# pangenome/sweepga

Hardware: AMD Instinct MI355X
Metric: PAF mappings/sec through plane-sweep+scaffold filter, 1/2/4/8 MI355X (higher is better)
Workload: dtype u32 coordinates, f64 scores; 1 GPU; BASELINE.json configs[3] (synthetic 100 M mappings across 10 k (q,t) groups, 100-genome pangenome shape; S-pan in SURVEY.md 8d): 100000000 mappings per GPU over 9900 genome-pair groups (100 single-chromosome genomes), pipeline=default; flags=(defaults), mappings_per_gpu=100000000, groups_per_gpu=9900

## Files before the change

### sweepga_amd/csrc/swg_pair.hip

```cpp
#include <cmath>
#include <type_traits>

#include "swg_scaffold_internal.h"

namespace swg_scaf {
namespace {

constexpr uint32_t PAIR_CELL = WALK_CHUNK;
constexpr uint32_t PAIR_S_MAX = 1024, PAIR_M_MAX = 4096, PAIR_L_MAX = 32768, PAIR_XL_MAX = uint32_t(1) << 18;
constexpr uint32_t PAIR_XL_CELLS = PAIR_XL_MAX / PAIR_CELL;
constexpr uint32_t PAIR_HASH_MAX = 65536;
constexpr uint32_t PF_NOT_GROUPED = 1, PF_RUN_OVERFLOW = 2, PF_TOO_LONG = 4, PF_FALLBACK = 8;

struct PairRun {
  uint32_t a, n;
};
struct PairInfo {
  uint32_t m;
  uint32_t m_plus;
  uint32_t M;
  uint32_t first_alive;
  uint32_t first_mem[2];
  uint32_t q, t;
};
struct PairSum {
  uint32_t n_pass;
  uint32_t n_kept;
  uint32_t minmem;
  uint32_t base;
};
struct PairCounters {
  uint32_t n_runs;
  uint32_t flags;
  uint32_t n_class[4];
  uint32_t n_chunks;
  uint32_t n_long;
  unsigned long long n_alive, n_members, n_heads, n_kept, n_out;
};

__device__ __forceinline__ void lds_barrier() {
  __builtin_amdgcn_fence(__ATOMIC_RELEASE, "wavefront");
  __builtin_amdgcn_s_waitcnt(0xc07f);
  __builtin_amdgcn_s_barrier();
  __builtin_amdgcn_fence(__ATOMIC_ACQUIRE, "wavefront");
}

template <int NT>
__device__ __forceinline__ uint32_t block_excl_sum(uint32_t v, uint32_t* ws, uint32_t* total) {
  const int lane = threadIdx.x & 63, w = threadIdx.x >> 6;
  uint32_t inc = v;
#pragma unroll
  for (int d = 1; d < 64; d <<= 1) {
    const uint32_t t = __shfl_up(inc, d, 64);
    if (lane >= d) inc += t;
  }
  if (NT == 64) {
    *total = __shfl(inc, 63, 64);
    return inc - v;
  }
  lds_barrier();
  if (lane == 63) ws[w] = inc;
  lds_barrier();
  uint32_t off = 0, tot = 0;
#pragma unroll
  for (int k = 0; k < NT / 64; ++k) {
    const uint32_t x = ws[k];
    off += k < w ? x : 0u;
// ... 132 lines not shown
    uint32_t h = (uint32_t)((key * 0x9e3779b97f4a7c15ull) >> 32) & tmask;
    for (;;) {
      const unsigned long long old = atomicCAS(&table[h], ~0ull, key);
      if (old == ~0ull) break;
      if (old == key) {
        atomicOr(&C->flags, PF_NOT_GROUPED);
        break;
      }
      h = (h + 1) & tmask;
    }
  }
  unsigned long long mk[4];
#pragma unroll
  for (int c = 0; c < 4; ++c) {
    mk[c] = __ballot(cls == c);
    if (lane == 0) s_cnt[wv][c] = (uint32_t)__popcll(mk[c]);
  }
  __syncthreads();
  if (threadIdx.x < 4) {
    const int c = threadIdx.x;
    const uint32_t tot = s_cnt[0][c] + s_cnt[1][c] + s_cnt[2][c] + s_cnt[3][c];
    s_base[c] = tot ? atomicAdd(&C->n_class[c], tot) : 0u;
  }
  __syncthreads();
  if (cls >= 0) {
    uint32_t o = s_base[cls];
    for (int w2 = 0; w2 < wv; ++w2) o += s_cnt[w2][cls];
    const unsigned long long m = cls == 0 ? mk[0] : (cls == 1 ? mk[1] : (cls == 2 ? mk[2] : mk[3]));
    class_list[(size_t)cls * cap + o + (uint32_t)__popcll(m & ((1ull << lane) - 1ull))] = k;
  }
}

constexpr int ORDER_NT = 1024, ORDER_BINS = 256;
__global__ __launch_bounds__(ORDER_NT) void pair_order_kernel(const PairRun* __restrict__ runs, uint32_t* __restrict__ class_list, uint32_t cap,
                                                              uint32_t* __restrict__ tmp, uint32_t cap_tmp,
                                                              const PairCounters* __restrict__ C) {
  __shared__ uint32_t bin_at[ORDER_BINS];
  const int tid = threadIdx.x, cls = 2 + (int)blockIdx.x;
  if (C->flags) return;
  const uint32_t cnt = C->n_class[cls];
  if (cnt < 2u || cnt > cap_tmp || cnt > cap) return;
  const uint32_t lo = cls == 2 ? PAIR_M_MAX : PAIR_L_MAX, width = (cls == 2 ? PAIR_L_MAX : PAIR_XL_MAX) - lo;
  uint32_t* const list = class_list + (size_t)cls * cap;
  uint32_t* const t = tmp + (size_t)blockIdx.x * cap_tmp;
  auto bin_of = [&](uint32_t len) -> uint32_t {
    const uint32_t b = (uint32_t)(((uint64_t)(len - lo - 1u) * ORDER_BINS) / width);
    return (uint32_t)ORDER_BINS - 1u - (b < (uint32_t)ORDER_BINS ? b : (uint32_t)ORDER_BINS - 1u);
  };
  for (int b = tid; b < ORDER_BINS; b += ORDER_NT) bin_at[b] = 0u;
  __syncthreads();
  for (uint32_t i = tid; i < cnt; i += ORDER_NT) {
    const uint32_t k = list[i];
    t[i] = k;
    atomicAdd(&bin_at[bin_of(runs[k].n)], 1u);
  }
  __syncthreads();
  if (tid < 64) {
    constexpr int PER = ORDER_BINS / 64;
    uint32_t v[PER], s = 0;
#pragma unroll
    for (int j = 0; j < PER; ++j) {
      v[j] = bin_at[tid * PER + j];
      s += v[j];
    }
    uint32_t inc = s;
#pragma unroll
    for (int d = 1; d < 64; d <<= 1) {
      const uint32_t x = __shfl_up(inc, d, 64);
      if (tid >= d) inc += x;
    }
    uint32_t o = inc - s;
#pragma unroll
    for (int j = 0; j < PER; ++j) {
      bin_at[tid * PER + j] = o;
      o += v[j];
    }
  }
  __syncthreads();
  for (uint32_t i = tid; i < cnt; i += ORDER_NT) {
    const uint32_t k = t[i];
    list[atomicAdd(&bin_at[bin_of(runs[k].n)], 1u)] = k;
  }
}

__global__ __launch_bounds__(256) void pair_hash_kernel(uint32_t n, const uint32_t* __restrict__ q_id, const uint32_t* __restrict__ t_id,
                                                        unsigned long long* __restrict__ table, uint32_t tmask,
                                                        uint32_t* __restrict__ count, uint32_t* __restrict__ slot_of) {
  const uint32_t i = blockIdx.x * 256u + threadIdx.x;
  if (i >= n) return;
  const unsigned long long key = (((unsigned long long)q_id[i] << 32) | t_id[i]) + 1ull;
  uint32_t h = (uint32_t)((key * 0x9e3779b97f4a7c15ull) >> 32) & tmask;
  for (;;) {
    unsigned long long old = __hip_atomic_load(&table[h], __ATOMIC_RELAXED, __HIP_MEMORY_SCOPE_AGENT);
    if (old == 0ull) {
      old = atomicCAS(&table[h], 0ull, key);
      if (old == 0ull) old = key;
    }
    if (old == key) break;
    h = (h + 1) & tmask;
  }
  slot_of[i] = h;
  atomicAdd(&count[h], 1u);
}
__global__ __launch_bounds__(256) void pair_slots_kernel(uint32_t tsize, const uint32_t* __restrict__ count, uint32_t* __restrict__ start,
                                                         PairRun* __restrict__ runs, uint32_t* __restrict__ class_list, uint32_t cap,
                                                         PairCounters* __restrict__ C, uint32_t* __restrict__ cursor) {
  const uint32_t h = blockIdx.x * 256u + threadIdx.x;
  const uint32_t c = h < tsize ? count[h] : 0u;
  if (!c) return;
// ... 56 lines not shown
  uint32_t b = (uint32_t)f;
  const uint32_t top = nb - 1u;
  b = b < top ? b : top;
  return off + b;
}

struct PairSortArgs {
  const uint32_t *q_id, *t_id, *q_start, *q_end, *t_start, *t_end, *matches, *block_len;
  const double* identity;
  const uint8_t* strand;
  const uint8_t *alive_in, *member_in;
  uint64_t min_block;
  int keep_self;
  double min_identity;
  int check_degenerate;
  uint64_t max_gap;
  const PairRun* runs;
  const uint32_t* list;
  const uint32_t* perm;
  const uint32_t* orig;
  uint8_t* code;
  uint32_t *s_qs, *s_qe, *s_ts, *s_te, *s_m, *s_b, *s_idx, *pred;
  PairInfo* info;
  SpecBlock* chunks;
  uint32_t cap_chunks;
  int chunks_by_place;
  uint32_t* long_list;
  uint32_t cap_long;
  PairCounters* C;
  PairTable gl_first;
  const uint32_t* seq_genome_last;
};

__device__ void emit_chunks(const PairSortArgs& A, uint32_t rk_run, uint32_t a, uint32_t m, uint32_t m_plus, const uint32_t* cellmin, int n_cell) {
  uint32_t prev = NONE, count = 0, n_long = 0, prev2 = NONE;
  const bool mp_pending = m_plus > 0 && m_plus < m;
  auto for_starts = [&](auto&& f) {
    bool pend = mp_pending;
    for (int c = 0; c < n_cell; ++c) {
      const uint32_t v = cellmin[c];
      if (v == NONE) continue;
      if (pend && m_plus <= v) {
        if (m_plus < v) f(m_plus);
        pend = false;
      }
      f(v);
    }
    if (pend) f(m_plus);
  };
  for_starts([&](uint32_t v) {
    ++count;
    if (prev2 != NONE && v - prev2 >= LABEL_CAP_ELEMS) ++n_long;
    prev2 = v;
  });
  if (prev2 != NONE && m - prev2 >= LABEL_CAP_ELEMS) ++n_long;
  const uint32_t slot = A.chunks_by_place ? a / PAIR_CELL + 2u * rk_run : atomicAdd(&A.C->n_chunks, count);
  uint32_t lslot = n_long ? atomicAdd(&A.C->n_long, n_long) : 0u;
  if (slot + count > A.cap_chunks || (n_long && lslot + n_long > A.cap_long)) {
    atomicOr(&A.C->flags, PF_FALLBACK);
    return;
  }
  uint32_t k = 0;
  auto emit = [&](uint32_t b, uint32_t e) {
    SpecBlock d;
    d.bb = a + b;
    d.be = a + e;
    d.ue = d.be;
    d.pad = b >= m_plus ? 1u : 0u;
    if (e - b >= LABEL_CAP_ELEMS) A.long_list[lslot++] = slot + k;
    A.chunks[slot + k++] = d;
  };
  for_starts([&](uint32_t v) {
    if (prev != NONE) emit(prev, v);
    prev = v;
  });
  if (prev != NONE) emit(prev, m);
}
template <int NT, int E>
__device__ __forceinline__ void unit_starts(const uint32_t (&qs)[E], const uint32_t (&qe)[E], uint32_t mb, uint32_t base, uint32_t m_plus,
                                            uint64_t max_gap, uint64_t* ws64, uint32_t* cellmin, uint64_t* carry_max) {
  const uint32_t p0 = (uint32_t)threadIdx.x * E;
  uint64_t tmax = 0;
#pragma unroll
  for (int e = 0; e < E; ++e)
    if (p0 + e < mb) {
      const uint64_t c = ((uint64_t)(base + p0 + e >= m_plus ? 1u : 0u) << 32) | qe[e];
      tmax = c > tmax ? c : tmax;
    }
  uint64_t tot;
  uint64_t prev = block_excl_max<NT>(tmax, ws64, &tot);
  prev = prev > *carry_max ? prev : *carry_max;
#pragma unroll
  for (int e = 0; e < E; ++e)
    if (p0 + e < mb) {
      const uint32_t pa = base + p0 + e;
      uint64_t lim = (prev & 0xffffffffull) + max_gap;
      if (lim < max_gap) lim = ~0ull;
      if (pa == 0 || pa == m_plus || (uint64_t)qs[e] > lim) atomicMin(&cellmin[pa / PAIR_CELL], pa);
      const uint64_t c = ((uint64_t)(pa >= m_plus ? 1u : 0u) << 32) | qe[e];
      prev = c > prev ? c : prev;
    }
  *carry_max = tot > *carry_max ? tot : *carry_max;
}
template <int E>
__device__ __forceinline__ void read_block(const uint32_t* lds, uint32_t (&out)[E]) {
  static_assert(E % 4 == 0, "whole 16-byte reads");
  const uint4* v = reinterpret_cast<const uint4*>(lds) + (size_t)threadIdx.x * (E / 4);
#pragma unroll
  for (int j = 0; j < E / 4; ++j) {
// ... 26 lines not shown
  constexpr int CAP = NT * ES, NREC = NT * ER, MAXB = 16, H = 8;
  constexpr int NCELL = (NREC + (int)PAIR_CELL - 1) / (int)PAIR_CELL;
  static_assert(ER <= 32 && ER % H == 0 && ES % 4 == 0 && NREC <= 65536, "record masks are 32 bits wide, indices 16");
  static_assert(NBIN >= 2 && NBIN <= 4096, "each strand needs a coarse bin of its own (the members are ordered strand first)");
  constexpr size_t O_K = 0, O_I = O_K + (size_t)CAP * 4, O_RR = O_I + (size_t)CAP * sizeof(IT), O_CNT = lds_align_up(O_RR + (size_t)CAP * 2, 4),
                   O_BINS = O_CNT + (size_t)NBK * 4, O_BLO = O_BINS + (size_t)NBIN * 4, O_CELL = O_BLO + (size_t)(MAXB + 1) * 4,
                   O_WS64 = lds_align_up(O_CELL + (size_t)NCELL * 4, 8), O_WS = O_WS64 + (size_t)(NT / 64 + 1) * 8,
                   O_SH = O_WS + (size_t)(NT / 64 + 1) * 4;
  static_assert(O_SH + 13 * 4 <= pair_sort_lds_bytes<NT, ES, ER, NBK, NBIN, PERM>(), "LDS block of the work-group");
  static_assert(O_CNT - O_I >= (size_t)CAP * 4 && O_I % 16 == 0, "B1 holds CAP words, read 16 bytes at a time");
  uint32_t* const K = reinterpret_cast<uint32_t*>(lds_raw + O_K);
  IT* const I = reinterpret_cast<IT*>(lds_raw + O_I);
  uint16_t* const RR = reinterpret_cast<uint16_t*>(lds_raw + O_RR);
  uint32_t* const B0 = K;
  uint32_t* const B1 = reinterpret_cast<uint32_t*>(lds_raw + O_I);
  uint32_t* const cnt = reinterpret_cast<uint32_t*>(lds_raw + O_CNT);
  uint32_t* const bins = reinterpret_cast<uint32_t*>(lds_raw + O_BINS);
  uint32_t* const b_lo = reinterpret_cast<uint32_t*>(lds_raw + O_BLO);
  uint32_t* const cellmin = reinterpret_cast<uint32_t*>(lds_raw + O_CELL);
  uint64_t* const ws64 = reinterpret_cast<uint64_t*>(lds_raw + O_WS64);
  uint32_t* const ws = reinterpret_cast<uint32_t*>(lds_raw + O_WS);
  uint32_t* const sh_cnt = reinterpret_cast<uint32_t*>(lds_raw + O_SH);
  uint32_t* const sh_kmin = sh_cnt + 4;
  uint32_t* const sh_kmax = sh_cnt + 6;
  uint32_t* const sh_first = sh_cnt + 8;
  uint32_t& sh_nb = sh_cnt[11];
  uint32_t& sh_bad = sh_cnt[12];
#ifdef SWG_PAIR_TIMING
  unsigned long long pt_last = wall_clock64();
#endif
  const int tid = threadIdx.x;
  const PairRun run = A.runs[rk_run];
  const uint32_t a = run.a, n = run.n;
  if (tid < 4) sh_cnt[tid] = 0;
  if (tid < 2) {
    sh_kmin[tid] = 0xffffffffu;
    sh_kmax[tid] = 0;
  }
  if (tid < 3) sh_first[tid] = NONE;
  if (tid == 0) sh_bad = 0;
  for (int c = tid; c < NCELL; c += NT) cellmin[c] = NONE;
  for (int b = tid; b < NBIN; b += NT) bins[b] = 0;
  lds_barrier();
  auto fresh_tid = [&]() -> uint32_t {
    uint32_t t = (uint32_t)tid;
    asm volatile("" : "+v"(t));
    return t;
  };
  uint32_t tid_v = (uint32_t)tid, n_v = n;
  auto rec_index = [&](int e) -> uint32_t {
    const uint32_t li = tid_v + (uint32_t)e * NT;
    const uint32_t lc = li < n_v ? li : 0u;
    return PERM ? A.perm[a + lc] : lc;
  };
  const uint32_t cb = PERM ? 0u : a;
  const uint32_t* c_qs = A.q_start + cb;
  const uint32_t* c_qe = A.q_end + cb;
  const uint32_t* c_ts = A.t_start + cb;
  const uint32_t* c_te = A.t_end + cb;
  const uint32_t* c_m = A.matches + cb;
  const uint32_t* c_b = A.block_len + cb;
  const uint8_t* c_st = A.strand + cb;
  const double* c_id = A.identity ? A.identity + cb : nullptr;
  const uint8_t* c_alive = A.alive_in ? A.alive_in + cb : nullptr;
  const uint8_t* c_member = A.member_in ? A.member_in + cb : nullptr;
  uint32_t* o_qs = A.s_qs + a;
// ... 437 lines not shown
      unit_starts<NT, ES>(qs_r, qe_r, mb, base, m_plus, A.max_gap, ws64, cellmin, &carry_max);
    }
    column(c_ts, B0, after_prev, B1, o_qe);
    lds_barrier();
    PT_STAMP(7);
    column(c_te, B1, after_prev, B0, o_ts);
    uint32_t ts_r[ES];
    read_block<ES>(B0, ts_r);
    lds_barrier();
    PT_STAMP(8);
    if (A.s_m) {
      column(c_m, B0, after_prev, B1, o_te);
    } else {
      store_column(B1, o_te);
    }
    {
      uint32_t te_r[ES];
      read_block<ES>(B1, te_r);
#pragma unroll
      for (int e = 0; e < ES; ++e) degenerate |= (uint32_t)tid * ES + e < mb && ts_r[e] >= te_r[e];
    }
    PT_STAMP(9);
    if (A.s_m) {
      lds_barrier();
      column(c_b, B1, after_prev, B0, o_m);
      lds_barrier();
      PT_STAMP(10);
      store_column(B1, o_b);
    }
    base += mb;
    PT_STAMP(11);
  }
  if (A.check_degenerate && __any(degenerate) && (tid & 63) == 0) atomicOr(&A.C->flags, PF_FALLBACK);
  if (tid == 0) emit_chunks(A, rk_run, a, m, m_plus, cellmin, NCELL);
  PT_STAMP(12);
}

template <int NT, int E, int NBK>
constexpr size_t pair_sort_xl_lds_bytes() {
  return (size_t)NT * E * 12 + (size_t)NBK * 4 + 4096 * 4 + 129 * 4 + (size_t)PAIR_XL_CELLS * 4 + (size_t)(NT / 64 + 1) * 12 + 16 * 4 + 128;
}
template <int NT, int E, int NBK>
__device__ __forceinline__ void pair_sort_xl_body(const PairSortArgs& A, const uint32_t rk_run, char* lds_raw) {
  constexpr int CAP = NT * E;
  constexpr int NBIN = 4096, MAXB = 128, U = 8;
  constexpr size_t O_K = 0, O_QE = O_K + (size_t)CAP * 4, O_I = O_QE + (size_t)CAP * 4, O_CNT = O_I + (size_t)CAP * 4,
                   O_BINS = O_CNT + (size_t)NBK * 4, O_BLO = O_BINS + (size_t)NBIN * 4, O_CELL = O_BLO + (size_t)(MAXB + 1) * 4,
                   O_WS64 = lds_align_up(O_CELL + (size_t)PAIR_XL_CELLS * 4, 8), O_WS = O_WS64 + (size_t)(NT / 64 + 1) * 8,
                   O_SH = O_WS + (size_t)(NT / 64 + 1) * 4;
  static_assert(O_SH + 13 * 4 <= pair_sort_xl_lds_bytes<NT, E, NBK>(), "LDS block of the work-group");
  uint32_t* const K = reinterpret_cast<uint32_t*>(lds_raw + O_K);
  uint32_t* const QE = reinterpret_cast<uint32_t*>(lds_raw + O_QE);
  uint32_t* const I = reinterpret_cast<uint32_t*>(lds_raw + O_I);
  uint32_t* const cnt = reinterpret_cast<uint32_t*>(lds_raw + O_CNT);
  uint32_t* const bins = reinterpret_cast<uint32_t*>(lds_raw + O_BINS);
  uint32_t* const b_lo = reinterpret_cast<uint32_t*>(lds_raw + O_BLO);
  uint32_t* const cellmin = reinterpret_cast<uint32_t*>(lds_raw + O_CELL);
  uint64_t* const ws64 = reinterpret_cast<uint64_t*>(lds_raw + O_WS64);
  uint32_t* const ws = reinterpret_cast<uint32_t*>(lds_raw + O_WS);
  uint32_t* const sh_cnt = reinterpret_cast<uint32_t*>(lds_raw + O_SH);
  uint32_t* const sh_kmin = sh_cnt + 4;
  uint32_t* const sh_kmax = sh_cnt + 6;
  uint32_t* const sh_first = sh_cnt + 8;
  uint32_t& sh_nb = sh_cnt[11];
  uint32_t& sh_bad = sh_cnt[12];
#ifdef SWG_PAIR_TIMING
  unsigned long long pt_last = wall_clock64();
// ... 319 lines not shown
      }
#pragma unroll
      for (int e = 0; e < E; ++e) {
        const uint32_t p = (uint32_t)tid + (uint32_t)e * NT;
        if (p >= mb) continue;
        const uint32_t o = a + base + p, qs = K[p];
        QE[p] = qe[e];
        A.s_qs[o] = qs;
        A.s_idx[o] = a + li[e];
        A.pred[o] = NONE;
        A.s_qe[o] = qe[e];
        A.s_ts[o] = ts[e];
        A.s_te[o] = te[e];
        if (A.s_m) {
          A.s_m[o] = mm[e];
          A.s_b[o] = bb[e];
        }
        degenerate |= qs >= qe[e] || ts[e] >= te[e];
      }
    }
    __syncthreads();
    PT_STAMP(7);
    {
      uint32_t qs_r[E], qe_r[E];
      read_block<E>(K, qs_r);
      read_block<E>(QE, qe_r);
      unit_starts<NT, E>(qs_r, qe_r, mb, base, m_plus, A.max_gap, ws64, cellmin, &carry_max);
    }
    base += mb;
    __syncthreads();
    PT_STAMP(8);
  }
  if (A.check_degenerate && __any(degenerate) && (tid & 63) == 0) atomicOr(&A.C->flags, PF_FALLBACK);
  if (tid == 0) emit_chunks(A, rk_run, a, m, m_plus, cellmin, (int)PAIR_XL_CELLS);
  PT_STAMP(9);
}

template <int NT, int ES, int ER, int NBK, int NBIN, bool PERM>
__global__ __launch_bounds__(NT) void pair_sort_kernel(PairSortArgs A) {
  __shared__ __attribute__((aligned(16))) char raw[pair_sort_lds_bytes<NT, ES, ER, NBK, NBIN, PERM>()];
  pair_sort_body<NT, ES, ER, NBK, NBIN, PERM>(A, A.list[blockIdx.x], raw);
}
constexpr size_t PAIR_BIG_LDS = pair_sort_lds_bytes<1024, 16, 32, 4096, 1024, false>() > pair_sort_xl_lds_bytes<1024, 8, 4096>()
                                    ? pair_sort_lds_bytes<1024, 16, 32, 4096, 1024, false>()
                                    : pair_sort_xl_lds_bytes<1024, 8, 4096>();
static_assert(PAIR_BIG_LDS <= 160 * 1024, "LDS of a CU");
__global__ __launch_bounds__(1024) void pair_sort_big_kernel(PairSortArgs A, const uint32_t* __restrict__ list_xl, uint32_t n_xl) {
  __shared__ __attribute__((aligned(16))) char raw[PAIR_BIG_LDS];
  if (blockIdx.x < n_xl)
    pair_sort_xl_body<1024, 8, 4096>(A, list_xl[blockIdx.x], raw);
  else
    pair_sort_body<1024, 16, 32, 4096, 1024, false>(A, A.list[blockIdx.x - n_xl], raw);
}

__global__ __launch_bounds__(1024) void pair_totals_kernel(uint32_t n_runs, const PairInfo* __restrict__ info, const PairSum* __restrict__ sum,
                                                           const uint32_t* __restrict__ n_out_pair, PairCounters* __restrict__ C) {
  __shared__ unsigned long long part[16][4];
  unsigned long long v[4] = {0, 0, 0, 0};
  const bool finished = !(C->flags & PF_FALLBACK);
  for (uint32_t k = blockIdx.x * 1024u + threadIdx.x; k < n_runs; k += gridDim.x * 1024u) {
    const PairInfo pi = info[k];
    v[0] += pi.M;
    v[1] += pi.m;
    if (finished) {
      v[2] += pi.M ? sum[k].n_kept : 0u;
      v[3] += n_out_pair[k];
    }
  }
#pragma unroll
  for (int j = 0; j < 4; ++j) {
#pragma unroll
    for (int o = 32; o > 0; o >>= 1) v[j] += __shfl_xor(v[j], o, 64);
    if ((threadIdx.x & 63) == 0) part[threadIdx.x >> 6][j] = v[j];
  }
  __syncthreads();
// ... 986 lines not shown
  const uint32_t n = (uint32_t)n64;
  hipStream_t st = ctx->stream;
  uint64_t* key = swg_alloc<uint64_t>(ctx, n);
  uint64_t* key2 = swg_alloc<uint64_t>(ctx, n);
  uint32_t* val = swg_alloc<uint32_t>(ctx, n);
  uint32_t* val2 = swg_alloc<uint32_t>(ctx, n);
  uint32_t* c4[8];
  for (auto& p : c4) p = swg_alloc<uint32_t>(ctx, n);
  double* c_id = r->identity ? swg_alloc<double>(ctx, n) : nullptr;
  uint8_t* c_st = swg_alloc<uint8_t>(ctx, n);
  SWG_CHECK_ARENA(ctx);
  SWG_LAUNCH(ctx, "pair_group_key", pair_group_key_kernel<<<(n + 255) / 256, 256, 0, st>>>(n, r->q_id, r->t_id, r->n_seq, key, val));
  SWG_KERNEL_CHECK(ctx);
  SWG_TRY(swg_radix_sort_pairs(ctx, &key, &val, &key2, &val2, n, 0, key_bits));
  SWG_LAUNCH(ctx, "pair_group_gather", pair_group_gather_kernel<<<(n + 255) / 256, 256, 0, st>>>(n, val, r->q_id, r->t_id, r->q_start, r->q_end, r->t_start, r->t_end,
                                                                                       r->matches, r->block_len, r->identity, r->strand, c4[0], c4[1], c4[2],
                                                                                       c4[3], c4[4], c4[5], c4[6], c4[7], c_id, c_st));
  SWG_KERNEL_CHECK(ctx);
  *copy = *r;
  copy->q_id = c4[0]; copy->t_id = c4[1]; copy->q_start = c4[2]; copy->q_end = c4[3]; copy->t_start = c4[4]; copy->t_end = c4[5];
  copy->matches = c4[6]; copy->block_len = c4[7]; copy->identity = c_id; copy->strand = c_st;
  *perm_out = val;
  *ok = 1;
  return SWG_OK;
}
int pair_ungroup_results(swg_ctx* ctx, uint64_t n, const uint32_t* perm, const uint8_t* st, const uint32_t* ch, uint8_t* status_out, uint32_t* chain_out) {
  SWG_LAUNCH(ctx, "pair_ungroup", pair_ungroup_kernel<<<(unsigned)((n + 255) / 256), 256, 0, ctx->stream>>>((uint32_t)n, perm, st, ch, status_out, chain_out));
  SWG_KERNEL_CHECK(ctx);
  return SWG_OK;
}

namespace {

}

int pair_plan(swg_ctx* ctx, const swg_records* r, const swg_config* cfg, PairPlan* plan) {
  *plan = PairPlan{};
  if (!pair_path_wanted()) return SWG_OK;
  const uint64_t n64 = r->n;
  if (n64 < 2 || n64 >= (uint64_t(1) << 31)) return SWG_OK;
  const uint32_t n = (uint32_t)n64;
  hipStream_t st = ctx->stream;
  static const bool dbg = getenv("SWG_DEBUG") != nullptr;
  const swg_arena_mark mark0 = swg_arena_save(ctx);
  const bool by_hash = n <= PAIR_HASH_MAX;
  bool plain = cfg != nullptr;
  if (cfg) {
    const bool sf_limited = cfg->scaffold_filter_mode == SWG_MODE_ONE_TO_ONE || cfg->scaffold_filter_mode == SWG_MODE_ONE_TO_MANY ||
                            cfg->scaffold_max_per_query != 0 || cfg->scaffold_max_per_target != 0;
    const bool mf_limited = cfg->mapping_filter_mode == SWG_MODE_ONE_TO_ONE || cfg->mapping_filter_mode == SWG_MODE_ONE_TO_MANY ||
                            cfg->mapping_max_per_query != 0 || cfg->mapping_max_per_target != 0;
    plain = !sf_limited && !mf_limited && (cfg->scaffolds_only || cfg->scaffold_max_deviation == 0);
  }
  static const uint32_t per_pair_env = getenv("SWG_PAIR_MIN_AVG") && atoi(getenv("SWG_PAIR_MIN_AVG")) > 0 ? (uint32_t)atoi(getenv("SWG_PAIR_MIN_AVG")) : 0u;
  const uint32_t per_pair = per_pair_env ? per_pair_env : (plain ? 96u : 192u);
  const uint32_t cap = by_hash ? (n < 8192u ? n : 8192u) : (n / per_pair > 8192u ? n / per_pair : 8192u);
  uint32_t tsize = 1;
  while (tsize < 2 * (by_hash ? n : cap)) tsize <<= 1;
  PairCounters* C = nullptr;
  PairRun* runs = swg_alloc<PairRun>(ctx, cap);
  uint32_t* class_list = swg_alloc<uint32_t>(ctx, (size_t)4 * cap);
  uint32_t* perm = nullptr;
  if (by_hash) {
    char* z = static_cast<char*>(swg_arena_alloc(ctx, (size_t)tsize * 12 + sizeof(PairCounters) + 8));
    uint32_t* slot_of = swg_alloc<uint32_t>(ctx, n);
    uint32_t* start = swg_alloc<uint32_t>(ctx, tsize);
// ... 1 lines not shown
    SWG_CHECK_ARENA(ctx);
    unsigned long long* table = reinterpret_cast<unsigned long long*>(z);
    uint32_t* count = reinterpret_cast<uint32_t*>(z + (size_t)tsize * 8);
    C = reinterpret_cast<PairCounters*>(z + (size_t)tsize * 12);
    uint32_t* cursor = reinterpret_cast<uint32_t*>(z + (size_t)tsize * 12 + sizeof(PairCounters));
    SWG_HIP(ctx, hipMemsetAsync(z, 0, (size_t)tsize * 12 + sizeof(PairCounters) + 8, st));
    SWG_LAUNCH(ctx, "pair_hash", pair_hash_kernel<<<(n + 255) / 256, 256, 0, st>>>(n, r->q_id, r->t_id, table, tsize - 1, count, slot_of));
    SWG_LAUNCH(ctx, "pair_slots", pair_slots_kernel<<<(tsize + 255) / 256, 256, 0, st>>>(tsize, count, start, runs, class_list, cap, C, cursor));
    SWG_LAUNCH(ctx, "pair_perm", pair_perm_kernel<<<(n + 255) / 256, 256, 0, st>>>(n, slot_of, start, perm));
    SWG_KERNEL_CHECK(ctx);
  } else {
    C = swg_alloc<PairCounters>(ctx, 1);
    const uint32_t n_words = (n + 63) / 64;
    unsigned long long* bitmap = swg_alloc<unsigned long long>(ctx, n_words + 1);
    uint32_t* wcnt = swg_alloc<uint32_t>(ctx, n_words + 1);
    uint32_t* wpre = swg_alloc<uint32_t>(ctx, n_words + 1);
    uint32_t* starts = swg_alloc<uint32_t>(ctx, (size_t)cap + 2);
    unsigned long long* table = swg_alloc<unsigned long long>(ctx, tsize);
    uint64_t* d_nr = swg_alloc<uint64_t>(ctx, 1);
    static const bool order_knob = !(getenv("SWG_PAIR_ORDER") && atoi(getenv("SWG_PAIR_ORDER")) == 0);
    const uint32_t cap_tmp = n / PAIR_M_MAX + 1u < cap ? n / PAIR_M_MAX + 1u : cap;
    uint32_t* order_tmp = order_knob ? swg_alloc<uint32_t>(ctx, (size_t)2 * cap_tmp) : nullptr;
    SWG_CHECK_ARENA(ctx);
    SWG_HIP(ctx, hipMemsetAsync(C, 0, sizeof(PairCounters), st));
    SWG_HIP(ctx, hipMemsetAsync(table, 0xff, (size_t)tsize * 8, st));
    SWG_LAUNCH(ctx, "pair_boundary", pair_boundary_kernel<<<(n + 1023) / 1024, 256, 0, st>>>(n, r->q_id, r->t_id, bitmap, wcnt));
    SWG_KERNEL_CHECK(ctx);
    SWG_TRY(swg_exclusive_scan_u32(ctx, wcnt, wpre, n_words, d_nr));
    SWG_LAUNCH(ctx, "pair_runs", pair_starts_kernel<<<(n_words + 255) / 256, 256, 0, st>>>(n, n_words, bitmap, wpre, d_nr, cap, starts));
    SWG_KERNEL_CHECK(ctx);
    SWG_LAUNCH(ctx, "pair_runs", pair_runs_kernel<<<(cap + 255) / 256, 256, 0, st>>>(n, cap, d_nr, starts, r->q_id, r->t_id, table, tsize - 1, runs, class_list, C));
    SWG_KERNEL_CHECK(ctx);
    if (order_knob && n > PAIR_M_MAX) {
      SWG_LAUNCH(ctx, "pair_order", pair_order_kernel<<<2, ORDER_NT, 0, st>>>(runs, class_list, cap, order_tmp, cap_tmp, C));
      SWG_KERNEL_CHECK(ctx);
    }
  }
  uint64_t h[4];
  static_assert(sizeof(PairCounters) >= 32, "the first four words are read back");
  SWG_TRY(swg_read_scalars(ctx, reinterpret_cast<const uint64_t*>(C), h, 3));
  const uint32_t n_runs = (uint32_t)h[0], flags = (uint32_t)(h[0] >> 32);
  if (flags || n_runs == 0) {
    if (dbg) fprintf(stderr, "[swg] pair path: not applicable (%u runs, flags %u)\n", n_runs, flags);
    plan->not_grouped = !by_hash && (flags & (PF_NOT_GROUPED | PF_RUN_OVERFLOW)) && !(flags & PF_TOO_LONG);
    swg_arena_restore(ctx, mark0);
    return SWG_OK;
  }
  if ((uint64_t)n / n_runs > PAIR_L_MAX) {
    if (dbg) fprintf(stderr, "[swg] pair path: %u pairs of %llu records on average: left to the global-sort stage\n", n_runs, (unsigned long long)n / n_runs);
    swg_arena_restore(ctx, mark0);
    return SWG_OK;
  }
  plan->valid = 1;
  plan->by_hash = by_hash;
  plan->n_runs = n_runs;
  plan->ncls[0] = (uint32_t)h[1];
  plan->ncls[1] = (uint32_t)(h[1] >> 32);
  plan->ncls[2] = (uint32_t)h[2];
  plan->ncls[3] = (uint32_t)(h[2] >> 32);
  plan->cap = cap;
  plan->counters = C;
  plan->runs = runs;
  plan->class_list = class_list;
  plan->perm = perm;
  if (dbg)
    fprintf(stderr, "[swg] pair path: %u pairs (%u / %u / %u / %u by size class)%s\n", n_runs, plan->ncls[0], plan->ncls[1], plan->ncls[2],
            plan->ncls[3], by_hash ? ", found through the hash table" : "");
  return SWG_OK;
}

int scaffold_stage_pairs(swg_ctx* ctx, const swg_records* r, const swg_config* cfg, const uint8_t* alive, const uint8_t* member,
                         bool sweep_assumed_identity, uint8_t* status_out, uint32_t* chain_out, swg_stats* stats, int* taken,
                         const PairPlan* plan_in) {
  *taken = 0;
  PairPlan own;
  if (!plan_in) {
    SWG_TRY(pair_plan(ctx, r, cfg, &own));
    plan_in = &own;
  }
  if (!plan_in->valid) return SWG_OK;
  uint64_t kq, kt;
  if (cfg->scaffold_filter_mode == SWG_MODE_ONE_TO_ONE) {
    kq = kt = 1;
  } else {
    kq = cfg->scaffold_max_per_query ? cfg->scaffold_max_per_query : SWG_K_INF;
    kt = cfg->scaffold_max_per_target ? cfg->scaffold_max_per_target : SWG_K_INF;
  }
  const bool limited = kq != SWG_K_INF || kt != SWG_K_INF;
  const bool rescue = !cfg->scaffolds_only && cfg->scaffold_max_deviation != 0;
  const bool need_wid = limited || !(cfg->min_scaffold_identity <= 0.0);
  const uint32_t n = (uint32_t)r->n;
  hipStream_t st = ctx->stream;
// ... 39 lines not shown
    SWG_HIP(ctx, hipMemsetAsync(chain_out, 0, (size_t)n * sizeof(uint32_t), st));
    SWG_HIP(ctx, hipMemsetAsync(status_out, 0, n, st));
  }
  SWG_HIP(ctx, hipMemsetAsync(n_out_pair, 0, (size_t)n_runs * sizeof(uint32_t), st));
  if (!by_hash) {
    SWG_HIP(ctx, hipMemsetAsync(chunks, 0, (size_t)cap_chunks * sizeof(SpecBlock), st));
    SWG_HIP(ctx, hipMemsetD32Async(reinterpret_cast<hipDeviceptr_t>(&C->n_chunks), (int)cap_chunks, 1, st));
  }
  PairSortArgs SA{};
  SA.q_id = r->q_id; SA.t_id = r->t_id; SA.q_start = r->q_start; SA.q_end = r->q_end; SA.t_start = r->t_start; SA.t_end = r->t_end;
  SA.matches = r->matches; SA.block_len = r->block_len; SA.identity = r->identity; SA.strand = r->strand;
  SA.alive_in = alive; SA.member_in = member;
  SA.min_block = cfg->min_block_length; SA.keep_self = cfg->keep_self; SA.min_identity = cfg->min_identity;
  SA.check_degenerate = sweep_assumed_identity ? 1 : 0;
  SA.max_gap = cfg->scaffold_gap;
  SA.runs = runs;
  SA.perm = perm;
  SA.orig = plan_in->orig;
  SA.code = code; SA.s_qs = s_qs; SA.s_qe = s_qe; SA.s_ts = s_ts; SA.s_te = s_te; SA.s_m = need_wid ? s_m : nullptr; SA.s_b = need_wid ? s_b : nullptr; SA.s_idx = s_idx; SA.pred = pred;
  SA.info = info; SA.chunks = chunks; SA.cap_chunks = cap_chunks; SA.chunks_by_place = by_hash ? 0 : 1; SA.long_list = long_list; SA.cap_long = cap_long; SA.C = C; SA.gl_first = gl_first; SA.seq_genome_last = r->seq_genome_last;
  if (by_hash) {
    for (int c = 2; c >= 0; --c) {
      if (!ncls[c]) continue;
      SA.list = class_list + (size_t)c * cap;
      if (c == 0)
        SWG_LAUNCH_N(ctx, "pair_sort_ps", 0, pair_sort_kernel<64, 16, 16, 256, 64, true><<<ncls[c], 64, 0, st>>>(SA));
      else if (c == 1)
        SWG_LAUNCH_N(ctx, "pair_sort_pm", 0, pair_sort_kernel<256, 16, 16, 1024, 64, true><<<ncls[c], 256, 0, st>>>(SA));
      else
        SWG_LAUNCH_N(ctx, "pair_sort_pl", 0, pair_sort_kernel<1024, 8, 32, 2048, 1024, true><<<ncls[c], 1024, 0, st>>>(SA));
      SWG_KERNEL_CHECK(ctx);
    }
  } else {
    if (ncls[2] + ncls[3]) {
      SA.list = class_list + (size_t)2 * cap;
      SWG_LAUNCH_N(ctx, "pair_sort_big", 0, pair_sort_big_kernel<<<ncls[2] + ncls[3], 1024, 0, st>>>(SA, class_list + (size_t)3 * cap, ncls[3]));
      SWG_KERNEL_CHECK(ctx);
    }
    for (int c = 1; c >= 0; --c) {
      if (!ncls[c]) continue;
      SA.list = class_list + (size_t)c * cap;
      if (c == 0)
        SWG_LAUNCH_N(ctx, "pair_sort_s", 0, pair_sort_kernel<64, 16, 16, 256, 64, false><<<ncls[c], 64, 0, st>>>(SA));
      else
        SWG_LAUNCH_N(ctx, "pair_sort_m", 0, pair_sort_kernel<256, 16, 16, 1024, 64, false><<<ncls[c], 256, 0, st>>>(SA));
      SWG_KERNEL_CHECK(ctx);
    }
  }
  if (!by_hash) {
    SWG_LAUNCH(ctx, "pair_gate", pair_gate_kernel<<<1, 64, 0, st>>>(C));
    SWG_KERNEL_CHECK(ctx);
  }
  const bool long_possible = ncls[2] + ncls[3] > 0;
  const uint32_t* lab_m = need_wid ? s_m : nullptr;
  const uint32_t* lab_b = need_wid ? s_b : nullptr;
  auto short_leg = [&]() -> int {
    SWG_TRY(pair_walk_launch(ctx, cap_chunks, &C->n_chunks, chunks, s_qs, s_qe, s_ts, s_te, cfg->scaffold_gap, bps, pred));
    return SWG_OK;
  };
  auto short_label = [&]() -> int {
    return pair_label_launch(ctx, cap_chunks, &C->n_chunks, chunks, pred, s_qs, s_qe, s_ts, s_te, lab_m, lab_b, cfg->min_scaffold_length,
                             cfg->min_scaffold_identity, hd, ok_head, head_rec, &C->n_heads);
  };
  auto long_walk = [&](hipStream_t ls) -> int {
    SWG_TRY(pair_walk_long_launch(ctx, ls, cap_long, &C->n_long, long_list, chunks, n, s_qs, s_qe, s_ts, s_te, cfg->scaffold_gap, bps, pred,
                                  &C->flags, PF_FALLBACK));
    if (!by_hash) {
      swg_on_stream on(ctx, ls);
      SWG_LAUNCH(ctx, "pair_gate", pair_gate_kernel<<<1, 64, 0, ls>>>(C));
// ... 147 lines not shown
    SWG_KERNEL_CHECK(ctx);
    SWG_TRY(swg_exclusive_scan_u32(ctx, sizes, sizes, n_runs, nullptr));
    SWG_LAUNCH(ctx, "pair_number", pair_base_kernel<<<rb, EW, 0, st>>>(n_runs, val, sizes, sum));
    SWG_KERNEL_CHECK(ctx);
  }
  {
    const unsigned gb = n_runs < (unsigned)ctx->num_cu * 16 ? n_runs : (unsigned)ctx->num_cu * 16;
    if (fin) {
      const unsigned cu = (unsigned)ctx->num_cu;
      if (ncls[2] + ncls[3]) {
        const uint32_t nb = ncls[2] + ncls[3];
        SWG_LAUNCH(ctx, "pair_renumber", pair_out_kernel<1024, 16384><<<nb < cu * 8 ? nb : cu * 8, 1024, 0, st>>>(
                                             ncls[3], class_list + (size_t)3 * cap, ncls[2], class_list + (size_t)2 * cap, runs, info, sum, s_idx, fin,
                                             chain_out, status_out, C));
        SWG_KERNEL_CHECK(ctx);
      }
      if (ncls[1]) {
        SWG_LAUNCH(ctx, "pair_renumber", pair_out_kernel<256, 4096><<<ncls[1] < cu * 16 ? ncls[1] : cu * 16, 256, 0, st>>>(
                                             0u, nullptr, ncls[1], class_list + (size_t)1 * cap, runs, info, sum, s_idx, fin, chain_out, status_out, C));
        SWG_KERNEL_CHECK(ctx);
      }
      if (ncls[0]) {
        SWG_LAUNCH(ctx, "pair_renumber", pair_out_kernel<64, 1024><<<ncls[0] < cu * 64 ? ncls[0] : cu * 64, 64, 0, st>>>(
                                             0u, nullptr, ncls[0], class_list, runs, info, sum, s_idx, fin, chain_out, status_out, C));
        SWG_KERNEL_CHECK(ctx);
      }
    } else {
      SWG_LAUNCH(ctx, "pair_renumber", pair_renumber_kernel<<<gb, EW, 0, st>>>(n_runs, runs, sum, chain_out, C, perm));
      SWG_KERNEL_CHECK(ctx);
    }
  }
  SWG_LAUNCH(ctx, "pair_totals", pair_totals_kernel<<<(n_runs + 4095) / 4096 < 64u ? (n_runs + 4095) / 4096 : 64u, 1024, 0, st>>>(n_runs, info, sum, n_out_pair, C));
  SWG_KERNEL_CHECK(ctx);
  uint64_t hc[9];
  static_assert(sizeof(PairCounters) == 72, "PairCounters is read back as nine words");
  SWG_TRY(swg_read_scalars(ctx, reinterpret_cast<const uint64_t*>(C), hc, 9));
  const uint32_t flags2 = (uint32_t)(hc[0] >> 32);
  if (flags2) {
    if (dbg) fprintf(stderr, "[swg] pair path: left on the device's word (flags %u): the global-sort path takes the call\n", flags2);
    swg_arena_restore(ctx, mark0);
    return SWG_OK;
  }
#ifdef SWG_PAIR_TIMING
  {
    unsigned long long ht[16];
    (void)hipMemcpyFromSymbol(ht, HIP_SYMBOL(g_pair_t), sizeof ht);
    fprintf(stderr, "[swg] pair_sort phases (100 MHz ticks summed over work-groups):");
    for (int k = 0; k < 13; ++k) fprintf(stderr, " %d:%llu", k, ht[k]);
    fprintf(stderr, "\n");
    unsigned long long z[16] = {0};
    (void)hipMemcpyToSymbol(HIP_SYMBOL(g_pair_t), z, sizeof z);
    (void)hipMemcpyFromSymbol(ht, HIP_SYMBOL(g_fin_t), sizeof ht);
    fprintf(stderr, "[swg] pair_finish phases:");
    for (int k = 0; k < 8; ++k) fprintf(stderr, " %d:%llu", k, ht[k]);
    fprintf(stderr, "\n");
    (void)hipMemcpyToSymbol(HIP_SYMBOL(g_fin_t), z, sizeof z);
  }
#endif
  if (stats) {
    stats->n_retained = hc[4];
    stats->n_swept = hc[5];
    stats->n_chains = hc[6];
    stats->n_chains_kept = hc[7];
    stats->n_out = hc[8];
  }
  *taken = 1;
  return SWG_OK;
}

}
```

### sweepga_amd/csrc/swg_scaffold_internal.h

```cpp
#pragma once
#include <cstdio>
#include <cstdlib>
#include <vector>

#include "swg_log.h"
#include "swg_pipeline.h"

namespace swg_scaf {

constexpr int EW = 256;
constexpr uint32_t NONE = 0xffffffffu;
inline unsigned nblk(uint64_t n) { return (unsigned)((n + EW - 1) / EW); }

static __global__ __launch_bounds__(EW) void fill_u32_kernel(uint64_t n, uint32_t* __restrict__ p, uint32_t v) {
  uint64_t i = (uint64_t)blockIdx.x * EW + threadIdx.x;
  if (i < n) p[i] = v;
}
static __global__ __launch_bounds__(EW) void fill_u64_kernel(uint64_t n, uint64_t* __restrict__ p, uint64_t v) {
  uint64_t i = (uint64_t)blockIdx.x * EW + threadIdx.x;
  if (i < n) p[i] = v;
}
static __global__ __launch_bounds__(EW) void iota_u32_kernel(uint64_t n, uint32_t* __restrict__ p) {
  uint64_t i = (uint64_t)blockIdx.x * EW + threadIdx.x;
  if (i < n) p[i] = (uint32_t)i;
// ... 147 lines not shown
  uint64_t* d_tot = nullptr;
  const SpecBlock* chunks = nullptr;
  uint64_t n_chunks = 0;
  const uint8_t* big_member = nullptr;
  const uint8_t* span_big = nullptr;
};

int chain_predecessors(swg_ctx* ctx, const swg_records* r, const uint8_t* alive, const uint8_t* member, uint64_t max_gap,
                       int pos_bits, ChainBuild* out, ChainWork* work, const uint32_t* q_order, uint64_t n_alive,
                       const swg_key_ends* slots);
int chain_table_build(swg_ctx* ctx, const swg_records* r, const uint8_t* alive, uint64_t min_len, double min_ident,
                      bool genome_pair_major, ChainBuild* out, const ChainWork& work);
inline int build_chains(swg_ctx* ctx, const swg_records* r, const uint8_t* alive, const uint8_t* member, uint64_t max_gap,
                        uint64_t min_len, double min_ident, int pos_bits, bool genome_pair_major, ChainBuild* out,
                        const uint32_t* q_order = nullptr, uint64_t n_alive = ~0ull, const swg_key_ends* slots = nullptr) {
  ChainWork W;
  SWG_TRY(chain_predecessors(ctx, r, alive, member, max_gap, pos_bits, out, &W, q_order, n_alive, slots));
  if (out->M == 0 || out->m == 0) return SWG_OK;
  return chain_table_build(ctx, r, alive, min_len, min_ident, genome_pair_major, out, W);
}

int scaffold_sweep_and_number(swg_ctx* ctx, const ChainTable& T, uint32_t n_seq, const uint32_t* seq_genome2,
                              uint32_t n_g2, int mode, uint64_t max_q, uint64_t max_t, double thr, int scoring,
                              int pos_bits, uint8_t* C_kept, uint32_t* C_num, uint64_t* n_kept_out);

int scaffold_sweep_segments(swg_ctx* ctx, uint64_t nc, const uint64_t* seg, int seg_bits, const uint32_t* qs, const uint32_t* qe,
                            const uint32_t* ts, const uint32_t* te, const double* wid, uint64_t kq, uint64_t kt, double thr, int scoring,
                            int pos_bits, uint8_t* kept, const void* runs = nullptr, uint32_t n_runs = 0);

struct PairPlan {
  int valid = 0;
  bool by_hash = false;
  uint32_t n_runs = 0, ncls[4] = {0, 0, 0, 0}, cap = 0;
  void *counters = nullptr, *runs = nullptr, *class_list = nullptr, *perm = nullptr;
  bool not_grouped = false;
  const uint32_t* orig = nullptr;
};
int pair_group_records(swg_ctx* ctx, const swg_records* r, swg_records* copy, uint32_t** perm, int* ok);
int pair_ungroup_results(swg_ctx* ctx, uint64_t n, const uint32_t* perm, const uint8_t* st, const uint32_t* ch, uint8_t* status_out, uint32_t* chain_out);
int pair_plan(swg_ctx* ctx, const swg_records* r, const swg_config* cfg, PairPlan* plan);
int scaffold_stage_pairs(swg_ctx* ctx, const swg_records* r, const swg_config* cfg, const uint8_t* alive, const uint8_t* member,
                         bool sweep_assumed_identity, uint8_t* status_out, uint32_t* chain_out, swg_stats* stats, int* taken,
                         const PairPlan* plan = nullptr);

}
```

Baseline: 12.14 billion mappings/s.

## Route mid-size pairs to a 512-thread sort kernel and wave-parallelize chunk emission

Measured after the change: 12.64 billion mappings/s, median of 6. 1.04x the previous value.

```diff
diff --git a/sweepga_amd/csrc/swg_pair.hip b/sweepga_amd/csrc/swg_pair.hip
--- a/sweepga_amd/csrc/swg_pair.hip
+++ b/sweepga_amd/csrc/swg_pair.hip
@@ -10,6 +10,9 @@
 constexpr uint32_t PAIR_S_MAX = 1024, PAIR_M_MAX = 4096, PAIR_L_MAX = 32768, PAIR_XL_MAX = uint32_t(1) << 18;
 constexpr uint32_t PAIR_XL_CELLS = PAIR_XL_MAX / PAIR_CELL;
 constexpr uint32_t PAIR_HASH_MAX = 65536;
+constexpr uint32_t PAIR_MX_MAX = 16384, PAIR_MX_CUT_DEFAULT = 8192;
+constexpr uint32_t ORDER_BIN_L = 128;
+constexpr uint32_t ORDERED = 0x80000000u;
 constexpr uint32_t PF_NOT_GROUPED = 1, PF_RUN_OVERFLOW = 2, PF_TOO_LONG = 4, PF_FALLBACK = 8;
 
 struct PairRun {
@@ -33,6 +36,8 @@
   uint32_t n_runs;
   uint32_t flags;
   uint32_t n_class[4];
+  uint32_t n_above;
+  uint32_t pad_;
   uint32_t n_chunks;
   uint32_t n_long;
   unsigned long long n_alive, n_members, n_heads, n_kept, n_out;
@@ -231,21 +236,30 @@
 }
 
 constexpr int ORDER_NT = 1024, ORDER_BINS = 256;
+static_assert((PAIR_L_MAX - PAIR_M_MAX) % ORDER_BIN_L == 0 && (PAIR_L_MAX - PAIR_M_MAX) / ORDER_BIN_L <= (uint32_t)ORDER_BINS &&
+                  (PAIR_XL_MAX - PAIR_L_MAX) % (uint32_t)ORDER_BINS == 0 && PAIR_M_MAX % ORDER_BIN_L == 0,
+              "whole bins, a bin boundary at every multiple of ORDER_BIN_L");
 __global__ __launch_bounds__(ORDER_NT) void pair_order_kernel(const PairRun* __restrict__ runs, uint32_t* __restrict__ class_list, uint32_t cap,
-                                                              uint32_t* __restrict__ tmp, uint32_t cap_tmp,
-                                                              const PairCounters* __restrict__ C) {
+                                                              uint32_t* __restrict__ tmp, uint32_t cap_tmp, uint32_t cut,
+                                                              PairCounters* __restrict__ C) {
   __shared__ uint32_t bin_at[ORDER_BINS];
   const int tid = threadIdx.x, cls = 2 + (int)blockIdx.x;
   if (C->flags) return;
   const uint32_t cnt = C->n_class[cls];
-  if (cnt < 2u || cnt > cap_tmp || cnt > cap) return;
-  const uint32_t lo = cls == 2 ? PAIR_M_MAX : PAIR_L_MAX, width = (cls == 2 ? PAIR_L_MAX : PAIR_XL_MAX) - lo;
   uint32_t* const list = class_list + (size_t)cls * cap;
+  if (cnt > cap_tmp || cnt > cap) return;
+  if (cnt < 2u) {
+    if (cls == 2 && tid == 0) C->n_above = ORDERED | (cnt && runs[list[0]].n > cut ? 1u : 0u);
+    return;
+  }
+  const uint32_t lo = cls == 2 ? PAIR_M_MAX : PAIR_L_MAX;
+  const uint32_t bw = cls == 2 ? ORDER_BIN_L : (PAIR_XL_MAX - PAIR_L_MAX) / (uint32_t)ORDER_BINS;
   uint32_t* const t = tmp + (size_t)blockIdx.x * cap_tmp;
   auto bin_of = [&](uint32_t len) -> uint32_t {
-    const uint32_t b = (uint32_t)(((uint64_t)(len - lo - 1u) * ORDER_BINS) / width);
+    const uint32_t b = (len - lo - 1u) / bw;
     return (uint32_t)ORDER_BINS - 1u - (b < (uint32_t)ORDER_BINS ? b : (uint32_t)ORDER_BINS - 1u);
   };
+  const uint32_t cut_bin = (uint32_t)ORDER_BINS - (cut > lo ? (cut - lo) / bw : 0u);
   for (int b = tid; b < ORDER_BINS; b += ORDER_NT) bin_at[b] = 0u;
   __syncthreads();
   for (uint32_t i = tid; i < cnt; i += ORDER_NT) {
@@ -271,9 +285,11 @@
     uint32_t o = inc - s;
 #pragma unroll
     for (int j = 0; j < PER; ++j) {
+      if (cls == 2 && (uint32_t)(tid * PER + j) == cut_bin) C->n_above = ORDERED | o;
       bin_at[tid * PER + j] = o;
       o += v[j];
     }
+    if (cls == 2 && cut_bin == (uint32_t)ORDER_BINS && tid == 63) C->n_above = ORDERED | o;
   }
   __syncthreads();
   for (uint32_t i = tid; i < cnt; i += ORDER_NT) {
@@ -396,49 +412,90 @@
   const uint32_t* seq_genome_last;
 };
 
-__device__ void emit_chunks(const PairSortArgs& A, uint32_t rk_run, uint32_t a, uint32_t m, uint32_t m_plus, const uint32_t* cellmin, int n_cell) {
-  uint32_t prev = NONE, count = 0, n_long = 0, prev2 = NONE;
-  const bool mp_pending = m_plus > 0 && m_plus < m;
-  auto for_starts = [&](auto&& f) {
-    bool pend = mp_pending;
-    for (int c = 0; c < n_cell; ++c) {
-      const uint32_t v = cellmin[c];
-      if (v == NONE) continue;
-      if (pend && m_plus <= v) {
-        if (m_plus < v) f(m_plus);
-        pend = false;
-      }
-      f(v);
-    }
-    if (pend) f(m_plus);
+__device__ __forceinline__ void emit_chunks(const PairSortArgs& A, uint32_t rk_run, uint32_t a, uint32_t m, uint32_t m_plus, const uint32_t* cellmin, int n_cell) {
+  const int lane = threadIdx.x & 63;
+  const unsigned long long below = (1ull << lane) - 1ull;
+  uint32_t n_start = 0, n_lt = 0, before_mp = NONE, last = NONE;
+  bool mp_is_start = false;
+  for (int c0 = 0; c0 < n_cell; c0 += 64) {
+    const uint32_t v = c0 + lane < n_cell ? cellmin[c0 + lane] : NONE;
+    const unsigned long long mask = __ballot(v != NONE);
+    if (!mask) continue;
+    const unsigned long long lt = __ballot(v != NONE && v < m_plus);
+    mp_is_start |= __ballot(v == m_plus) != 0ull;
+    n_start += (uint32_t)__popcll(mask);
+    n_lt += (uint32_t)__popcll(lt);
+    if (lt) before_mp = (uint32_t)__shfl((int)v, 63 - __clzll(lt), 64);
+    last = (uint32_t)__shfl((int)v, 63 - __clzll(mask), 64);
+  }
+  const bool mp_ins = m_plus > 0 && m_plus < m && !mp_is_start;
+  const uint32_t count = n_start + (mp_ins ? 1u : 0u);
+  if (count == 0) return;
+  auto begin_of = [&](uint32_t v, unsigned long long mask, uint32_t carry) -> uint32_t {
+    const unsigned long long lower = mask & below;
+    const uint32_t pv = (uint32_t)__shfl((int)v, lower ? 63 - __clzll(lower) : 0, 64);
+    uint32_t b = lower ? pv : carry;
+    if (mp_ins && m_plus < v && (b == NONE || b < m_plus)) b = m_plus;
+    return b;
   };
-  for_starts([&](uint32_t v) {
-    ++count;
-    if (prev2 != NONE && v - prev2 >= LABEL_CAP_ELEMS) ++n_long;
-    prev2 = v;
-  });
-  if (prev2 != NONE && m - prev2 >= LABEL_CAP_ELEMS) ++n_long;
-  const uint32_t slot = A.chunks_by_place ? a / PAIR_CELL + 2u * rk_run : atomicAdd(&A.C->n_chunks, count);
-  uint32_t lslot = n_long ? atomicAdd(&A.C->n_long, n_long) : 0u;
+  const bool mp_chunk = mp_ins && before_mp != NONE;
+  const bool mp_long = mp_chunk && m_plus - before_mp >= LABEL_CAP_ELEMS;
+  const uint32_t last_b = mp_ins && (last == NONE || last < m_plus) ? m_plus : last;
+  const bool last_long = m - last_b >= LABEL_CAP_ELEMS;
+  uint32_t n_long = (mp_long ? 1u : 0u) + (last_long ? 1u : 0u), n_long_lt = 0;
+  {
+    uint32_t carry = NONE;
+    for (int c0 = 0; c0 < n_cell; c0 += 64) {
+      const uint32_t v = c0 + lane < n_cell ? cellmin[c0 + lane] : NONE;
+      const unsigned long long mask = __ballot(v != NONE);
+      if (!mask) continue;
+      const uint32_t b = begin_of(v, mask, carry);
+      const bool lf = v != NONE && b != NONE && v - b >= LABEL_CAP_ELEMS;
+      n_long += (uint32_t)__popcll(__ballot(lf));
+      n_long_lt += (uint32_t)__popcll(__ballot(lf && v < m_plus));
+      carry = (uint32_t)__shfl((int)v, 63 - __clzll(mask), 64);
+    }
+  }
+  uint32_t slot = 0, lslot = 0;
+  if (lane == 0) {
+    slot = A.chunks_by_place ? a / PAIR_CELL + 2u * rk_run : atomicAdd(&A.C->n_chunks, count);
+    lslot = n_long ? atomicAdd(&A.C->n_long, n_long) : 0u;
+  }
+  slot = (uint32_t)__shfl((int)slot, 0, 64);
+  lslot = (uint32_t)__shfl((int)lslot, 0, 64);
   if (slot + count > A.cap_chunks || (n_long && lslot + n_long > A.cap_long)) {
-    atomicOr(&A.C->flags, PF_FALLBACK);
+    if (lane == 0) atomicOr(&A.C->flags, PF_FALLBACK);
     return;
   }
-  uint32_t k = 0;
-  auto emit = [&](uint32_t b, uint32_t e) {
+  auto emit = [&](uint32_t k, uint32_t b, uint32_t e, bool is_long, uint32_t lpos) {
     SpecBlock d;
     d.bb = a + b;
     d.be = a + e;
     d.ue = d.be;
     d.pad = b >= m_plus ? 1u : 0u;
-    if (e - b >= LABEL_CAP_ELEMS) A.long_list[lslot++] = slot + k;
-    A.chunks[slot + k++] = d;
+    if (is_long) A.long_list[lslot + lpos] = slot + k;
+    A.chunks[slot + k] = d;
   };
-  for_starts([&](uint32_t v) {
-    if (prev != NONE) emit(prev, v);
-    prev = v;
-  });
-  if (prev != NONE) emit(prev, m);
+  uint32_t carry = NONE, base = 0, lbase = 0;
+  for (int c0 = 0; c0 < n_cell; c0 += 64) {
+    const uint32_t v = c0 + lane < n_cell ? cellmin[c0 + lane] : NONE;
+    const unsigned long long mask = __ballot(v != NONE);
+    if (!mask) continue;
+    const uint32_t b = begin_of(v, mask, carry);
+    const bool lf = v != NONE && b != NONE && v - b >= LABEL_CAP_ELEMS;
+    const unsigned long long lmask = __ballot(lf);
+    if (v != NONE && b != NONE) {
+      const uint32_t k = base + (uint32_t)__popcll(mask & below) + (mp_ins && v > m_plus ? 1u : 0u) - 1u;
+      emit(k, b, v, lf, lbase + (uint32_t)__popcll(lmask & below) + (mp_long && v > m_plus ? 1u : 0u));
+    }
+    base += (uint32_t)__popcll(mask);
+    lbase += (uint32_t)__popcll(lmask);
+    carry = (uint32_t)__shfl((int)v, 63 - __clzll(mask), 64);
+  }
+  if (lane == 0) {
+    if (mp_chunk) emit(n_lt - 1u, before_mp, m_plus, mp_long, n_long_lt);
+    emit(count - 1u, last_b, m, last_long, n_long - 1u);
+  }
 }
 template <int NT, int E>
 __device__ __forceinline__ void unit_starts(const uint32_t (&qs)[E], const uint32_t (&qe)[E], uint32_t mb, uint32_t base, uint32_t m_plus,
@@ -531,6 +588,10 @@
   const int tid = threadIdx.x;
   const PairRun run = A.runs[rk_run];
   const uint32_t a = run.a, n = run.n;
+  if (n > (uint32_t)NREC) {
+    if (tid == 0) atomicOr(&A.C->flags, PF_FALLBACK);
+    return;
+  }
   if (tid < 4) sh_cnt[tid] = 0;
   if (tid < 2) {
     sh_kmin[tid] = 0xffffffffu;
@@ -1034,7 +1095,7 @@
     PT_STAMP(11);
   }
   if (A.check_degenerate && __any(degenerate) && (tid & 63) == 0) atomicOr(&A.C->flags, PF_FALLBACK);
-  if (tid == 0) emit_chunks(A, rk_run, a, m, m_plus, cellmin, NCELL);
+  if (tid < 64) emit_chunks(A, rk_run, a, m, m_plus, cellmin, NCELL);
   PT_STAMP(12);
 }
 
@@ -1420,7 +1481,7 @@
     PT_STAMP(8);
   }
   if (A.check_degenerate && __any(degenerate) && (tid & 63) == 0) atomicOr(&A.C->flags, PF_FALLBACK);
-  if (tid == 0) emit_chunks(A, rk_run, a, m, m_plus, cellmin, (int)PAIR_XL_CELLS);
+  if (tid < 64) emit_chunks(A, rk_run, a, m, m_plus, cellmin, (int)PAIR_XL_CELLS);
   PT_STAMP(9);
 }
 
@@ -1429,6 +1490,12 @@
   __shared__ __attribute__((aligned(16))) char raw[pair_sort_lds_bytes<NT, ES, ER, NBK, NBIN, PERM>()];
   pair_sort_body<NT, ES, ER, NBK, NBIN, PERM>(A, A.list[blockIdx.x], raw);
 }
+template <>
+__global__ __launch_bounds__(512) __attribute__((amdgpu_waves_per_eu(4))) void pair_sort_kernel<512, 16, 32, 2048, 1024, false>(PairSortArgs A) {
+  __shared__ __attribute__((aligned(16))) char raw[pair_sort_lds_bytes<512, 16, 32, 2048, 1024, false>()];
+  pair_sort_body<512, 16, 32, 2048, 1024, false>(A, A.list[blockIdx.x], raw);
+}
+static_assert(2 * pair_sort_lds_bytes<512, 16, 32, 2048, 1024, false>() <= 160 * 1024, "two work-groups in the LDS of a CU");
 constexpr size_t PAIR_BIG_LDS = pair_sort_lds_bytes<1024, 16, 32, 4096, 1024, false>() > pair_sort_xl_lds_bytes<1024, 8, 4096>()
                                     ? pair_sort_lds_bytes<1024, 16, 32, 4096, 1024, false>()
                                     : pair_sort_xl_lds_bytes<1024, 8, 4096>();
@@ -2481,6 +2548,26 @@
 
 namespace {
 
+}
+
+static_assert(PAIR_MX_MAX == 512 * 32 && PAIR_MX_MAX % ORDER_BIN_L == 0 && PAIR_MX_CUT_DEFAULT % ORDER_BIN_L == 0 && PAIR_MX_CUT_DEFAULT <= 512 * 16,
+              "NT x ER of pair_sort_mx; the default inside its NT x ES");
+static uint32_t pair_mx_cut() {
+  static const uint32_t cut = [] {
+    const char* e = getenv("SWG_PAIR_MX_MAX");
+    if (!e) return PAIR_MX_CUT_DEFAULT;
+    char* end = nullptr;
+    const long v = strtol(e, &end, 10);
+    if (end == e || *end != '\0' || v < 0 || v > (long)PAIR_MX_MAX) {
+      fprintf(stderr, "[swg] SWG_PAIR_MX_MAX=%s is not a number from 0 to %u: the default of %u is used\n", e, PAIR_MX_MAX, PAIR_MX_CUT_DEFAULT);
+      return PAIR_MX_CUT_DEFAULT;
+    }
+    const uint32_t c = (uint32_t)v / ORDER_BIN_L * ORDER_BIN_L;
+    const uint32_t cut = c > PAIR_M_MAX ? c : 0u;
+    if (getenv("SWG_DEBUG")) fprintf(stderr, "[swg] SWG_PAIR_MX_MAX=%s: pair_sort_mx takes pairs of up to %u records\n", e, cut);
+    return cut;
+  }();
+  return cut;
 }
 
 int pair_plan(swg_ctx* ctx, const swg_records* r, const swg_config* cfg, PairPlan* plan) {
@@ -2548,13 +2635,13 @@
     SWG_LAUNCH(ctx, "pair_runs", pair_runs_kernel<<<(cap + 255) / 256, 256, 0, st>>>(n, cap, d_nr, starts, r->q_id, r->t_id, table, tsize - 1, runs, class_list, C));
     SWG_KERNEL_CHECK(ctx);
     if (order_knob && n > PAIR_M_MAX) {
-      SWG_LAUNCH(ctx, "pair_order", pair_order_kernel<<<2, ORDER_NT, 0, st>>>(runs, class_list, cap, order_tmp, cap_tmp, C));
+      SWG_LAUNCH(ctx, "pair_order", pair_order_kernel<<<2, ORDER_NT, 0, st>>>(runs, class_list, cap, order_tmp, cap_tmp, pair_mx_cut(), C));
       SWG_KERNEL_CHECK(ctx);
     }
   }
   uint64_t h[4];
-  static_assert(sizeof(PairCounters) >= 32, "the first four words are read back");
-  SWG_TRY(swg_read_scalars(ctx, reinterpret_cast<const uint64_t*>(C), h, 3));
+  static_assert(offsetof(PairCounters, n_above) == 24, "the first four words are read back: the counts and pair_order's cut");
+  SWG_TRY(swg_read_scalars(ctx, reinterpret_cast<const uint64_t*>(C), h, 4));
   const uint32_t n_runs = (uint32_t)h[0], flags = (uint32_t)(h[0] >> 32);
   if (flags || n_runs == 0) {
     if (dbg) fprintf(stderr, "[swg] pair path: not applicable (%u runs, flags %u)\n", n_runs, flags);
@@ -2574,6 +2661,11 @@
   plan->ncls[1] = (uint32_t)(h[1] >> 32);
   plan->ncls[2] = (uint32_t)h[2];
   plan->ncls[3] = (uint32_t)(h[2] >> 32);
+  const uint32_t above = (uint32_t)h[3];
+  if (pair_mx_cut() && (above & ORDERED) && (above & ~ORDERED) <= plan->ncls[2]) {
+    plan->cut = pair_mx_cut();
+    plan->n_above = above & ~ORDERED;
+  }
   plan->cap = cap;
   plan->counters = C;
   plan->runs = runs;
@@ -2679,9 +2771,16 @@
       SWG_KERNEL_CHECK(ctx);
     }
   } else {
-    if (ncls[2] + ncls[3]) {
+    const uint32_t n_above = plan_in->cut ? plan_in->n_above : ncls[2], n_mx = ncls[2] - n_above;
+    if (dbg && ncls[2]) fprintf(stderr, "[swg] pair_sort: %u pairs under pair_sort_big, %u under pair_sort_mx (cut %u)\n", n_above + ncls[3], n_mx, plan_in->cut);
+    if (n_above + ncls[3]) {
       SA.list = class_list + (size_t)2 * cap;
-      SWG_LAUNCH_N(ctx, "pair_sort_big", 0, pair_sort_big_kernel<<<ncls[2] + ncls[3], 1024, 0, st>>>(SA, class_list + (size_t)3 * cap, ncls[3]));
+      SWG_LAUNCH_N(ctx, "pair_sort_big", 0, pair_sort_big_kernel<<<n_above + ncls[3], 1024, 0, st>>>(SA, class_list + (size_t)3 * cap, ncls[3]));
+      SWG_KERNEL_CHECK(ctx);
+    }
+    if (n_mx) {
+      SA.list = class_list + (size_t)2 * cap + n_above;
+      SWG_LAUNCH_N(ctx, "pair_sort_mx", 0, pair_sort_kernel<512, 16, 32, 2048, 1024, false><<<n_mx, 512, 0, st>>>(SA));
       SWG_KERNEL_CHECK(ctx);
     }
     for (int c = 1; c >= 0; --c) {
@@ -2895,9 +2994,9 @@
   }
   SWG_LAUNCH(ctx, "pair_totals", pair_totals_kernel<<<(n_runs + 4095) / 4096 < 64u ? (n_runs + 4095) / 4096 : 64u, 1024, 0, st>>>(n_runs, info, sum, n_out_pair, C));
   SWG_KERNEL_CHECK(ctx);
-  uint64_t hc[9];
-  static_assert(sizeof(PairCounters) == 72, "PairCounters is read back as nine words");
-  SWG_TRY(swg_read_scalars(ctx, reinterpret_cast<const uint64_t*>(C), hc, 9));
+  uint64_t hc[10];
+  static_assert(sizeof(PairCounters) == 80 && offsetof(PairCounters, n_alive) == 40, "PairCounters is read back as ten words");
+  SWG_TRY(swg_read_scalars(ctx, reinterpret_cast<const uint64_t*>(C), hc, 10));
   const uint32_t flags2 = (uint32_t)(hc[0] >> 32);
   if (flags2) {
     if (dbg) fprintf(stderr, "[swg] pair path: left on the device's word (flags %u): the global-sort path takes the call\n", flags2);
@@ -2921,11 +3020,11 @@
   }
 #endif
   if (stats) {
-    stats->n_retained = hc[4];
-    stats->n_swept = hc[5];
-    stats->n_chains = hc[6];
-    stats->n_chains_kept = hc[7];
-    stats->n_out = hc[8];
+    stats->n_retained = hc[5];
+    stats->n_swept = hc[6];
+    stats->n_chains = hc[7];
+    stats->n_chains_kept = hc[8];
+    stats->n_out = hc[9];
   }
   *taken = 1;
   return SWG_OK;
diff --git a/sweepga_amd/csrc/swg_scaffold_internal.h b/sweepga_amd/csrc/swg_scaffold_internal.h
--- a/sweepga_amd/csrc/swg_scaffold_internal.h
+++ b/sweepga_amd/csrc/swg_scaffold_internal.h
@@ -203,6 +203,7 @@
   int valid = 0;
   bool by_hash = false;
   uint32_t n_runs = 0, ncls[4] = {0, 0, 0, 0}, cap = 0;
+  uint32_t n_above = 0, cut = 0;
   void *counters = nullptr, *runs = nullptr, *class_list = nullptr, *perm = nullptr;
   bool not_grouped = false;
   const uint32_t* orig = nullptr;
```
